# LANL-Bioinformatics/KWAGE

Hardware: AMD Instinct MI355X
Metric: G k-mer·sample bit-tests/sec (+ achieved HBM GB/s of the gather kernel in `roofline`) (higher is better)
Workload: dtype u32

## Files before the change

kwage_amd/csrc/engine.hip:

```cpp
#include <hip/hip_runtime.h>
#include <hip/hip_ext.h>

#include <algorithm>
#include <chrono>
#include <cmath>
#include <cstdio>
#include <cctype>
#include <cstring>
#include <new>
#include <string>
#include <thread>
#include <vector>

#include <unistd.h>

#include "host.hpp"
#include "engine_state.hpp"
#include "kernels.hpp"
#include "search_plan.hpp"

using namespace kwage;


struct TuningName { const char *name; int64_t Tuning::*field; };
static const TuningName TUNING_NAMES[] = {
	{"walk", &Tuning::walk}, {"walk_min_rows", &Tuning::walk_min_rows}, {"walk_max_kib", &Tuning::walk_max_kib}, {"walk_min_kib", &Tuning::walk_min_kib}, {"walk_tile_kib", &Tuning::walk_tile_kib},
	 {"walk_waves", &Tuning::walk_waves}, {"walk_one_wg_per_cu", &Tuning::walk_one_wg_per_cu},
	{"walk_bands", &Tuning::walk_bands}, {"walk_bands_min_gib", &Tuning::walk_bands_min_gib},
	{"and_vec", &Tuning::and_vec}, {"and_wide", &Tuning::and_wide}, {"and_wide_min_kib", &Tuning::and_wide_min_kib}, {"narrow", &Tuning::narrow}, {"force_segs", &Tuning::force_segs}, {"scores_form", &Tuning::scores_form},
	{"ee_refine", &Tuning::ee_refine}, {"refine_seg_rows", &Tuning::refine_seg_rows}, {"refine_min_rows", &Tuning::refine_min_rows}, {"refine_max_groups", &Tuning::refine_max_groups}, {"refine_unroll", &Tuning::refine_unroll}, {"refine_list_cap", &Tuning::refine_list_cap}, {"refine_static", &Tuning::refine_static}, {"screen_wpc", &Tuning::screen_wpc}, {"count_screen_wpc", &Tuning::count_screen_wpc}, {"count_screen_min_tiles", &Tuning::count_screen_min_tiles}, {"count_screen_check", &Tuning::count_screen_check}, {"count_trunc", &Tuning::count_trunc},
	{"count_walk", &Tuning::count_walk}, {"count_walk_wpc", &Tuning::count_walk_wpc}, {"count_walk_waves", &Tuning::count_walk_waves},
	{"count_walk_min_rows", &Tuning::count_walk_min_rows},
	{"hit_sort_host", &Tuning::hit_sort_host}, {"hit_copy_piece_kb", &Tuning::hit_copy_piece_kb}, {"shared_table_log2", &Tuning::shared_table_log2},
	{"ext_launch_events", &Tuning::ext_launch_events}, {"group_contiguous", &Tuning::group_contiguous}, {"group_placement_probe", &Tuning::group_placement_probe},
};

namespace kwage {

__global__ __launch_bounds__(KM_THREADS) void kmer_kernel(KmerArgs a)
{
	extern __shared__ __attribute__((aligned(16))) unsigned long long lds_tab[];
	__shared__ uint8_t codes[KM_THREADS + KWAGE_MAX_WORD_LEN];
	__shared__ uint32_t count, tile_base;

	const uint32_t q = a.chunk_q ? a.chunk_q[blockIdx.x] : blockIdx.x;
	const uint64_t t_begin = a.chunk_q ? a.chunk_t0[blockIdx.x] : 0;
	const uint64_t s0 = a.seq_off[q];
	const uint64_t len = a.seq_off[q + 1] - s0;
	const uint64_t npos = (len >= a.k) ? (len - a.k + 1) : 0;

	if(npos == 0){
		if(threadIdx.x == 0){ a.nkmer[q] = 0; a.qthr[q] = 0; }
		return;
// ... 26 lines not shown
{
	const uint32_t q = blockIdx.x / wgs_per_query, part = blockIdx.x % wgs_per_query;
	uint32_t *rq = rows + pos_off[q]*num_hash;
	const uint64_t n = (uint64_t)nkmer[q]*num_hash;
	for(uint64_t e = (uint64_t)part*blockDim.x + threadIdx.x; e < n; e += (uint64_t)wgs_per_query*blockDim.x){
		const uint32_t r = rq[e];
		uint32_t lo = 0, hi = map_len;
		while(lo < hi){
			const uint32_t mid = lo + (hi - lo)/2;
			if(map[mid] < r){ lo = mid + 1; } else { hi = mid; }
		}
		if(lo < map_len && map[lo] == r){ rq[e] = lo; }
		else{ rq[e] = 0; atomicAdd(missing, 1ull); }
	}
}

__global__ __launch_bounds__(SEARCH_THREADS) void and_refine_emit_kernel(SearchArgs a, RefineArgs ra)
{
	constexpr int B = 4;
	__shared__ WaveHitBuf hit_bufs[SEARCH_THREADS/WAVE];
	WaveHitBuf *hbuf = &hit_bufs[threadIdx.x >> 6];
	WaveHitState hst;
	const uint32_t lane = threadIdx.x & (WAVE - 1), l = lane & 7u, g = lane >> 3;
	const uint32_t n_clusters = refine_list_end(ra, 0);
	const uint32_t gw = __builtin_amdgcn_readfirstlane(blockIdx.x*(blockDim.x/WAVE) + (threadIdx.x >> 6));
	const uint32_t nw = gridDim.x*(blockDim.x/WAVE);
	for(uint64_t c0 = gw; c0 < n_clusters; c0 += (uint64_t)B*nw){
		RefineCluster cl[B];
		u32x4 m[B];
#pragma unroll
		for(int k = 0; k < B; ++k){
			const uint64_t ci = c0 + (uint64_t)k*nw;
			cl[k].q = REFINE_NONE;
			if(ci < n_clusters){ cl[k] = ra.clusters[ci]; }
		}
#pragma unroll
		for(int k = 0; k < B; ++k){
			const uint32_t groups = cl[k].kstep_groups & 0xFFu;
			m[k] = (u32x4)(0u);
			if(cl[k].q != REFINE_NONE && ((groups >> g) & 1u)){
				const uint32_t it = cl[k].first_item + __popc(groups & ((1u << g) - 1u));
				m[k] = reinterpret_cast<const u32x4*>(ra.masks)[(uint64_t)it*8 + l];
			}
		}
#pragma unroll
		for(int k = 0; k < B; ++k){
			if(cl[k].q == REFINE_NONE){ continue; }
			const uint32_t kstep = cl[k].kstep_groups >> 8;
			emit_masked_hits_buffered(a, hbuf, hst, cl[k].q, kstep*WAVE + lane, m[k], cl[k].n, (uint64_t)cl[k].q*a.runs_per_query + kstep);
		}
	}
	wave_hits_flush(a, hbuf, hst);
}

__global__ __launch_bounds__(256) void band_bucket_kernel(const uint32_t *__restrict__ rows, const uint64_t *__restrict__ pos_off, const uint32_t *__restrict__ nkmer,
                                                         uint32_t num_hash, uint32_t bands, uint32_t rows_per_band, uint32_t *__restrict__ loc, uint32_t *__restrict__ rows2)
{
// ... 328 lines not shown
}

int launch_count_combine(const SearchPlan &p, const SearchArgs &a, hipStream_t s, const StageEvents &ge)
{
	return by_planes(p.planes, [&](auto P) -> int {
		constexpr int PLANES = decltype(P)::value;
		constexpr size_t lds = (size_t)(COMBINE_WAVES/2)*PLANES*WAVE*16;
		int rc;
		if((rc = allow_dynamic_lds(count_combine_kernel<PLANES>, lds))){ return rc; }
		KW_GATHER_LAUNCH(ge, false, true, (count_combine_kernel<PLANES>), dim3(p.combine_wgs, a.n_queries), dim3(COMBINE_WAVES*WAVE), lds, s, a, p.seg_planes);
		return KWAGE_OK;
	});
}

int reserve_zeroed(DevBuf &buf, uint64_t bytes, hipStream_t s)
{
	if(bytes <= buf.cap){ return KWAGE_OK; }
	int rc = buf.reserve(bytes);
	if(rc){ return rc; }
	HIP_TRY(hipMemsetAsync(buf.p, 0, buf.cap, s));
	return KWAGE_OK;
}

int refine_setup(Slot *sl, const RefinePlan &r, hipStream_t gs, RefineArgs *out)
{
	int rc;
	RefineArgs &ra = *out;
	auto list = [](const ListPlan &l) { return RefineList{l.cap, l.stat, l.base, l.chunk}; };
	ra.seg_rows = r.seg_rows;
	ra.min_rows = r.min_rows;
	ra.max_groups = r.max_groups;
	ra.lc = list(r.lc);
	ra.li = list(r.li);
	ra.lu = list(r.lu);
	if((rc = sl->ref_counters.reserve(8*sizeof(uint32_t)))){ return rc; }
	if((rc = sl->ref_clusters.reserve(r.clusters*sizeof(RefineCluster)))){ return rc; }
	if((rc = sl->ref_masks.reserve(r.items*r.item_bytes))){ return rc; }
	if((rc = sl->ref_units.reserve(r.units*sizeof(RefineUnit)))){ return rc; }
	if(r.unit_bytes && (rc = sl->ref_slab.reserve(r.units*r.unit_bytes))){ return rc; }
	ra.counters = (uint32_t*)sl->ref_counters.p;
	ra.clusters = (RefineCluster*)sl->ref_clusters.p;
	ra.masks = (uint32_t*)sl->ref_masks.p;
	ra.units = (RefineUnit*)sl->ref_units.p;
	ra.slab = (uint32_t*)sl->ref_slab.p;
	HIP_TRY(hipMemsetAsync(ra.counters, 0, 8*sizeof(uint32_t), gs));
	sl->ref_base[0] = ra.lc.base; sl->ref_base[1] = ra.li.base; sl->ref_base[2] = ra.lu.base;
	sl->ref_cap[0] = ra.lc.cap; sl->ref_cap[1] = ra.li.cap; sl->ref_cap[2] = ra.lu.cap;
	ra.queue_batch = r.queue_batch;
	ra.check_every = r.check_every;
	return KWAGE_OK;
}

int count_walk_setup(Slot *sl, const SearchPlan &p, hipStream_t gs, CountWalkArgs *wa)
{
	int rc;
	wa->total_slots = p.total_slots;
	wa->per_wave = p.per_wave;
	wa->coltiles = p.chunks;
	if((rc = sl->cwalk_slab.reserve(p.exchange_bytes))){ return rc; }
	if((rc = reserve_zeroed(sl->cwalk_arrived, p.flags_bytes, gs))){ return rc; }
	wa->slab = (uint32_t*)sl->cwalk_slab.p;
	wa->arrived = (uint32_t*)sl->cwalk_arrived.p;
	wa->slot_off = nullptr; wa->kcut = nullptr;
	return KWAGE_OK;
}

uint32_t count_screen_blocks_per_cu(uint32_t planes, uint32_t nh)
{
	static int cache[3][5] = {};
	const int pi = (planes <= 7) ? 0 : (planes <= 10) ? 1 : 2, ni = (int)std::min(std::max(nh, 1u), 5u) - 1;
// ... 198 lines not shown
static const uint64_t SORT_SCRATCH_KEEP = 1ull << 30;

struct SearchOutcome {
	uint64_t staged_hits = 0;
	uint64_t n_hits = 0;
	uint64_t total_kmers = 0;
	float kmer_ms = 0, search_ms = 0;
	uint32_t launches = 0;
	char kernel_name[64] = "";
};

int enqueue_search_and_copy(Slot *sl)
{
	int rc;
	kwage_group *g = sl->g;
	kwage_batch *b = sl->b;
	const bool timing = (sl->flags & KWAGE_SEARCH_TIMING) != 0;
	const bool own = (sl->ext_hits == nullptr && sl->ext_cap == 0);
	const uint64_t cap = own ? sl->hit_cap : sl->ext_cap;
	kwage_hit *d_hits = own ? sl->d_hits : sl->ext_hits;
	if(b->n && g->num_columns){
		hipStream_t gs = g->ctx->gather_stream;
		if(sl->n_runs){ HIP_TRY(hipMemsetAsync(sl->runs.p, 0, sl->n_runs*sizeof(unsigned long long), sl->stream)); }
		HIP_TRY(hipEventRecord(sl->kmer_done, sl->stream));
		HIP_TRY(hipStreamWaitEvent(gs, sl->kmer_done, 0));
		if(sl->append && sl->append_reset){ HIP_TRY(hipMemsetAsync(sl->ext_count, 0, sizeof(uint64_t), gs)); }
		const bool ride = g->ctx->tune.ext_launch_events != 0;
		StageEvents ge;
		if(ride){ ge.start = timing ? sl->ev[2] : nullptr; ge.stop = sl->gather_done; }
		else if(timing){ HIP_TRY(hipEventRecord(sl->ev[2], gs)); }
		unsigned long long *hit_count = sl->append ? (unsigned long long*)sl->ext_count : (unsigned long long*)sl->d_counters;
		if((rc = launch_search_stage(sl, g, b, sl->lay, sl->threshold, sl->flags, d_hits, cap, hit_count, gs, ge))){ return rc; }
		if(!ride){ HIP_TRY(hipEventRecord(sl->gather_done, gs)); }
		HIP_TRY(hipStreamWaitEvent(sl->stream, sl->gather_done, 0));
		++sl->launches;
	}
	else if(sl->append && sl->append_reset){
		hipStream_t gs = g->ctx->gather_stream;
		HIP_TRY(hipMemsetAsync(sl->ext_count, 0, sizeof(uint64_t), gs));
		HIP_TRY(hipEventRecord(sl->gather_done, gs));
		HIP_TRY(hipStreamWaitEvent(sl->stream, sl->gather_done, 0));
	}
	if(sl->append){
		HIP_TRY(hipMemcpyAsync(sl->d_counters, sl->ext_count, sizeof(uint64_t), hipMemcpyDeviceToDevice, sl->stream));
	}
	else if(sl->ext_count){
// ... 172 lines not shown
			hipLaunchKernelGGL(count_nonzero_kernel, dim3((uint32_t)std::min<uint64_t>(2048, (n + 255)/256)), dim3(256), 0, ctx->stream,
			                   (const uint32_t*)bufs[j]->p, n, d + j);
		}
		e = hipGetLastError();
	}
	unsigned long long h[5] = {0, 0, 0, 0, 0};
	if(e == hipSuccess){ e = hipMemcpyAsync(h, d, sizeof(h), hipMemcpyDeviceToHost, ctx->stream); }
	if(e == hipSuccess){ e = hipStreamSynchronize(ctx->stream); }
	(void)hipFree(d);
	if(e != hipSuccess){ return fail(KWAGE_ERR_DEVICE, "kwage_ctx_scratch_nonzero: %s", hipGetErrorString(e)); }
	for(int j = 0; j < 5; ++j){ out[j] = h[j]; }
	return KWAGE_OK;
}

extern "C" int kwage_ctx_refine_stats(kwage_ctx *ctx, uint64_t out[8])
{
	if(!ctx || !out){ return fail(KWAGE_ERR_ARG, "kwage_ctx_refine_stats: NULL argument"); }
	for(int i = 0; i < 2; ++i){ if(ctx->slot[i].busy){ return fail(KWAGE_ERR_STATE, "kwage_ctx_refine_stats: a search is pending on this context"); } }
	int rc = set_device(ctx);
	if(rc){ return rc; }
	HIP_TRY(hipStreamSynchronize(ctx->gather_stream));
	for(int k = 0; k < 2; ++k){
		Slot *sl = &ctx->slot[k];
		uint32_t h[4] = {0, 0, 0, 0};
		if(sl->ref_counters.p){ HIP_TRY(hipMemcpy(h, sl->ref_counters.p, sizeof(h), hipMemcpyDeviceToHost)); }
		for(int j = 0; j < 3; ++j){ out[4*k + j] = std::min<uint64_t>((uint64_t)sl->ref_base[j] + h[j], sl->ref_cap[j]); }
		out[4*k + 3] = sl->ref_cap[2];
	}
	return KWAGE_OK;
}

namespace kwage {
hipStream_t ctx_stream(kwage_ctx *ctx) { return ctx->stream; }
int ctx_device(kwage_ctx *ctx) { return ctx->device; }
}

extern "C" int kwage_device_count(void)
{
	int n = 0;
	if(hipGetDeviceCount(&n) != hipSuccess){ return 0; }
	return n;
}

extern "C" int kwage_init(int device, kwage_ctx **out)
{
	if(!out){ return fail(KWAGE_ERR_ARG, "kwage_init: out is NULL"); }
// ... 610 lines not shown
```

kwage_amd/csrc/engine_state.hpp:

```cpp
#ifndef KWAGE_AMD_ENGINE_STATE_HPP
#define KWAGE_AMD_ENGINE_STATE_HPP

#include <hip/hip_runtime.h>

#include <algorithm>
#include <deque>
#include <memory>
#include <mutex>
#include <type_traits>
#include <vector>

#include "internal.h"
#include "tuning.hpp"

#define HIP_TRY(expr)                                                                          \
	do {                                                                                       \
		hipError_t _e = (expr);                                                                \
		if(_e != hipSuccess){                                                                  \
			return fail(KWAGE_ERR_DEVICE, "%s failed: %s (%s:%d)", #expr, hipGetErrorString(_e), \
			            __FILE__, __LINE__);                                                   \
		}                                                                                      \
	} while(0)

struct kwage_group;
// ... 183 lines not shown
	uint32_t *d_nkmer = nullptr, *d_qthr = nullptr;
	kwage_hit *d_hits = nullptr;
	uint64_t hit_cap = 0, head_bytes = 0;
	PinBuf h_stage;
	DevBuf sort_scratch;
	DevBuf runs;
	uint64_t n_runs = 0;
	uint32_t runs_per_query = 0;
	bool busy = false;
	kwage_group *g = nullptr;
	kwage_batch *b = nullptr;
	const KmerLayout *lay = nullptr;
	float threshold = 1.0f;
	uint32_t flags = 0;
	uint32_t launches = 0;
	char kernel_name[64] = "";
	DevBuf walk_or, walk_done;
	DevBuf band_rows, band_loc, band_or, band_state;
	DevBuf cwalk_slab, cwalk_arrived;
	DevBuf ref_counters, ref_clusters, ref_masks, ref_units, ref_slab;
	DevBuf trunc_dev;
	PinBuf trunc_host;
	uint32_t ref_base[3] = {0, 0, 0}, ref_cap[3] = {0, 0, 0};
	uint64_t staged_hits = 0;
	kwage_hit *ext_hits = nullptr;
	uint64_t ext_cap = 0;
	uint64_t *ext_count = nullptr;
	bool append = false, append_reset = false;
	uint32_t col_base = 0;
};

}

struct kwage_ctx {
	int device = -1;
	int ncu = 0;
	kwage::Tuning tune;
	hipStream_t stream = nullptr;
	hipStream_t gather_stream = nullptr;
	hipStream_t upload_stream = nullptr;
	kwage::Slot slot[2];
	kwage::DevBuf kmers;
	kwage::DevPool batch_pool;
	kwage::PinBuf load_pin[2];
	kwage::DevBuf load_dev[3];
	hipEvent_t load_done[3] = {nullptr, nullptr, nullptr};
// ... 169 lines not shown
```

kwage_amd/csrc/kernels.hpp:

```cpp
#ifndef KWAGE_AMD_KERNELS_HPP
#define KWAGE_AMD_KERNELS_HPP

#include <hip/hip_runtime.h>
#include <stdint.h>

#include "kwage_amd.h"
#include "kmer_device.hpp"
#include "tuning.hpp"

namespace kwage {

static constexpr int KM_THREADS = 256;
static constexpr uint32_t KM_LDS_SLOTS = 4096;
static constexpr uint32_t KM_CHUNK = 1024;
static constexpr uint64_t KM_EMPTY = ~0ull;


__device__ __forceinline__ uint32_t table_log2(uint64_t npos)
{
	uint32_t lg = 6;
	while((1ull << lg) < 2*npos){ ++lg; }
	return lg;
}

template <typename PTR>
__device__ __forceinline__ bool set_insert(PTR tab, uint32_t lg, uint64_t w)
{
	const uint64_t mask = (1ull << lg) - 1ull;
	uint64_t s = ((w * 0x9E3779B97F4A7C15ull) >> (64 - lg)) & mask;
	while(true){
// ... 399 lines not shown
	}
}

struct RefineUnit { uint32_t item, r0, r1, unit0, rq_lo, rq_hi, q, pad; };
struct RefineCluster {
	uint32_t q, kstep_groups, first_item, n;
	uint32_t first_unit, nseg, pad0, pad1;
};
static constexpr uint32_t REFINE_NONE = 0xFFFFFFFFu;

struct RefineList { uint32_t cap, stat, base, chunk; };
struct RefineArgs {
	uint32_t *counters;
	RefineCluster *clusters;
	uint32_t *masks;
	RefineUnit *units;
	uint32_t *slab;
	RefineList lc, li, lu;
	uint32_t seg_rows;
	uint32_t min_rows;
	uint32_t max_groups;
	uint32_t queue_batch;
	uint32_t check_every;
};

__device__ __forceinline__ uint32_t group_bits(uint64_t lanes)
{
	uint32_t g = 0;
#pragma unroll
	for(int k = 0; k < 8; ++k){ g |= ((lanes >> (8*k)) & 0xFFull) ? (1u << k) : 0u; }
	return g;
}

__device__ __forceinline__ uint32_t nth_set_bit(uint32_t bits, uint32_t j)
{
	for(uint32_t k = 0; k < j; ++k){ bits &= bits - 1; }
	return __ffs(bits) - 1;
}

struct RefineChunk { uint32_t next = 0, end = 0; };

__device__ __forceinline__ void refine_none_clusters(const RefineArgs &ra, uint32_t from, uint32_t to)
{
	to = min(to, ra.lc.cap);
	for(uint32_t i = from + (threadIdx.x & (WAVE - 1)); i < to; i += WAVE){ ra.clusters[i].q = REFINE_NONE; }
}
// ... 14 lines not shown
		uint32_t r = 0;
		if((threadIdx.x & (WAVE - 1)) == 0){ r = atomicAdd(ra.counters + which, want); }
		const uint64_t at = (uint64_t)ls.base + __builtin_amdgcn_readfirstlane(r);
		if(at + want > ls.cap){
			if(at < ls.cap){
				if(which == 0){ refine_none_clusters(ra, (uint32_t)at, ls.cap); } else if(which == 2){ refine_none_units(ra, (uint32_t)at, ls.cap); }
			}
			return REFINE_NONE;
		}
		ch.next = (uint32_t)at;
		ch.end = (uint32_t)at + want;
	}
	const uint32_t at = ch.next;
	ch.next += need;
	return at;
}

__device__ __forceinline__ uint32_t refine_list_end(const RefineArgs &ra, int which)
{
	const RefineList &ls = (which == 0) ? ra.lc : (which == 1) ? ra.li : ra.lu;
	return (uint32_t)min((uint64_t)ls.base + ra.counters[which], (uint64_t)ls.cap);
}

template <int VEC, int UNROLL>
__global__ __launch_bounds__(SEARCH_THREADS) void and_screen_kernel(SearchArgs a, RefineArgs ra)
{
	const uint32_t lane = threadIdx.x & (WAVE - 1);
	const uint64_t n_tiles = (uint64_t)a.n_queries*a.chunks;
	const uint32_t n_waves = gridDim.x*(blockDim.x/WAVE);
	const uint32_t gw = __builtin_amdgcn_readfirstlane(blockIdx.x*(blockDim.x/WAVE) + (threadIdx.x >> 6));
	__shared__ WaveHitBuf hit_bufs[SEARCH_THREADS/WAVE];
	WaveHitBuf *hbuf = &hit_bufs[threadIdx.x >> 6];
	WaveHitState hst;
	RefineChunk cc, ci, cu;
	cc.next = gw*ra.lc.stat; cc.end = cc.next + ra.lc.stat;
	ci.next = gw*ra.li.stat; ci.end = ci.next + ra.li.stat;
	cu.next = gw*ra.lu.stat; cu.end = cu.next + ra.lu.stat;
	bool lists_full = false;
	for(uint64_t tile = gw; tile < n_tiles; tile += n_waves){
		const uint32_t q = __builtin_amdgcn_readfirstlane((uint32_t)(tile / a.chunks));
		const uint32_t c = __builtin_amdgcn_readfirstlane((uint32_t)(tile % a.chunks));
		const uint32_t n = a.nkmer[q];
		if(n == 0){ continue; }
		const uint32_t nrows = n*a.num_hash;
		const uint64_t rq_off = a.pos_off[q]*a.num_hash;
		const uint32_t *rq = a.rows + rq_off;

		uint32_t unit[VEC];
		u32x4 acc[VEC];
#pragma unroll
		for(int v = 0; v < VEC; ++v){
			const uint32_t u = c*(WAVE*VEC) + v*WAVE + lane;
			const bool live = (u < a.units_per_row);
			unit[v] = live ? u : (a.units_per_row - 1);
			acc[v] = live ? reinterpret_cast<const u32x4*>(a.valid)[u] : (u32x4)(0u);
		}

		bool may_hand_over = !lists_full, gone = false;
		uint32_t i = 0;
		for(; i + UNROLL <= nrows; i += UNROLL){
// ... 5 lines not shown
#pragma unroll
				for(int v = 0; v < VEC; ++v){ x[u][v] = load16<true>(p + unit[v]); }
			}
#pragma unroll
			for(int u = 0; u < UNROLL; ++u){
#pragma unroll
				for(int v = 0; v < VEC; ++v){ acc[v] &= x[u][v]; }
			}
			uint32_t gb[VEC], ngroups = 0;
#pragma unroll
			for(int v = 0; v < VEC; ++v){
				gb[v] = group_bits(__ballot((acc[v].x | acc[v].y | acc[v].z | acc[v].w) != 0));
				ngroups += __popc(gb[v]);
			}
			if(ngroups == 0){ gone = true; break; }
			const uint32_t done = i + UNROLL;
			if(may_hand_over && ngroups <= ra.max_groups && nrows - done >= ra.min_rows && (done >= 2*UNROLL || nrows < 4*ra.seg_rows)){
				may_hand_over = false;
				const uint32_t nseg = (nrows - done + ra.seg_rows - 1)/ra.seg_rows;
				uint32_t nc = 0;
#pragma unroll
				for(int v = 0; v < VEC; ++v){ nc += gb[v] ? 1u : 0u; }
				const uint32_t nu = ngroups*nseg;
				const uint32_t c0 = refine_take(ra, 0, cc, nc);
				const uint32_t i0 = (c0 != REFINE_NONE) ? refine_take(ra, 1, ci, ngroups) : REFINE_NONE;
				const uint32_t u0 = (i0 != REFINE_NONE) ? refine_take(ra, 2, cu, nu) : REFINE_NONE;
				if(u0 == REFINE_NONE){
					if(c0 != REFINE_NONE){ refine_none_clusters(ra, c0, c0 + nc); }
					lists_full = true;
					continue;
				}
				uint32_t cidx = c0, ii = i0, all_groups = 0;
#pragma unroll
				for(int v = 0; v < VEC; ++v){
					all_groups |= gb[v] << (8*v);
					if(!gb[v]){ continue; }
					if(lane == 0){
						RefineCluster cl; cl.q = q; cl.kstep_groups = ((c*VEC + v) << 8) | gb[v]; cl.first_item = ii; cl.n = n;
						cl.first_unit = 0; cl.nseg = 0; cl.pad0 = 0; cl.pad1 = 0;
						ra.clusters[cidx] = cl;
					}
					const uint32_t k = lane >> 3;
					if((gb[v] >> k) & 1u){
						const uint32_t it = ii + __popc(gb[v] & ((1u << k) - 1u));
						reinterpret_cast<u32x4*>(ra.masks)[(uint64_t)it*8 + (lane & 7u)] = acc[v];
					}
					++cidx;
					ii += __popc(gb[v]);
				}
				for(uint32_t e = lane; e < nu; e += WAVE){
					const uint32_t j = e / nseg, sg = e % nseg;
					const uint32_t gpos = nth_set_bit(all_groups, j);
					RefineUnit un;
					un.item = i0 + j;
					un.r0 = done + sg*ra.seg_rows;
					un.r1 = min(nrows, un.r0 + ra.seg_rows);
					un.unit0 = c*(WAVE*VEC) + gpos*8u;
					un.rq_lo = (uint32_t)rq_off; un.rq_hi = (uint32_t)(rq_off >> 32);
					un.q = q; un.pad = 0;
					ra.units[u0 + e] = un;
				}
				gone = true;
				break;
			}
		}
		if(gone){ continue; }
		for(; i < nrows; ++i){
			const uint32_t r = rq[i];
			const u32x4 *p = reinterpret_cast<const u32x4*>(a.db + (uint64_t)r*a.stride);
#pragma unroll
			for(int v = 0; v < VEC; ++v){ acc[v] &= load16<true>(p + unit[v]); }
		}
#pragma unroll
		for(int v = 0; v < VEC; ++v){
			emit_masked_hits_buffered(a, hbuf, hst, q, unit[v], acc[v], n, (uint64_t)q*a.runs_per_query + c*VEC + v);
		}
	}
	wave_hits_flush(a, hbuf, hst);
	refine_none_clusters(ra, cc.next, cc.end);
	refine_none_units(ra, cu.next, cu.end);
}

template <int UNROLL>
__global__ __launch_bounds__(SEARCH_THREADS) void and_refine_kernel(SearchArgs a, RefineArgs ra)
{
	static_assert(UNROLL == 8 || UNROLL == 16, "eight or sixteen rows in flight");
	const uint32_t lane = threadIdx.x & (WAVE - 1), l = lane & 7u, sh = lane & ~7u;
	const uint32_t n_units = refine_list_end(ra, 2);
	const uint64_t gw = (uint64_t)blockIdx.x*(blockDim.x/WAVE) + (threadIdx.x >> 6);
	const uint64_t step = (uint64_t)gridDim.x*(blockDim.x/WAVE)*8;
	for(uint64_t base = gw*8; base < n_units; base += step){
		const uint64_t u = base + (lane >> 3);
		RefineUnit un;
		un.item = REFINE_NONE;
		if(u < n_units){ un = ra.units[u]; }
		bool on = (un.item != REFINE_NONE);
		uint32_t *M = ra.masks;
		u32x4 m = (u32x4)(0u);
		if(on){
			M = ra.masks + ((uint64_t)un.item*8 + l)*4;
#pragma unroll
			for(int d = 0; d < 4; ++d){ m[d] = __hip_atomic_load(M + d, __ATOMIC_RELAXED, __HIP_MEMORY_SCOPE_AGENT); }
		}
		on = on && (((uint32_t)(__ballot((m.x | m.y | m.z | m.w) != 0) >> sh) & 0xFFu) != 0);
		if(on){
			const uint32_t *rq = a.rows + (((uint64_t)un.rq_hi << 32) | un.rq_lo);
			const u32x4 *col = reinterpret_cast<const u32x4*>(a.db) + (un.unit0 + l);
			u32x4 acc = ~(u32x4)(0u);
			bool alive = true;
			for(uint32_t b = un.r0; alive && b < un.r1; b += 64){
				uint32_t idx[8];
#pragma unroll
				for(int k = 0; k < 8; ++k){ idx[k] = rq[min(b + 8u*k + l, un.r1 - 1)]; }
#pragma unroll
				for(int k = 0; k < 8; k += UNROLL/8){
					if(b + 8u*k >= un.r1){ break; }
					u32x4 x[UNROLL];
#pragma unroll
// ... 1081 lines not shown
```

kwage_amd/csrc/search_plan.hpp:

```cpp
#ifndef KWAGE_AMD_SEARCH_PLAN_HPP
#define KWAGE_AMD_SEARCH_PLAN_HPP

#include <algorithm>
#include <cmath>
#include <cstdint>
#include <cstdio>

#include "internal.h"
#include "tuning.hpp"

namespace kwage {

inline uint32_t planes_for(uint64_t max_count)
{
	uint32_t bits = 1;
	while(bits < 32 && (max_count >> bits) != 0){ ++bits; }
	return (bits <= 7) ? 7 : (bits <= 10) ? 10 : (bits <= 14) ? 14 : (bits <= 20) ? 20 : 32;
}

struct Segments { uint32_t segs, seg_kmers; };
inline Segments choose_segments(uint64_t n_queries, uint32_t chunks, uint64_t max_kmers, uint64_t max_segs, int64_t force_segs)
{
	static const uint64_t TARGET_TILES = 2048, MIN_SEG_KMERS = 64;
	Segments s = {1, (uint32_t)std::max<uint64_t>(max_kmers, 1)};
	uint64_t want = 1;
	if(force_segs > 0){ want = (uint64_t)force_segs; }
	else{
		const uint64_t tiles = n_queries*chunks;
		if(tiles >= TARGET_TILES || max_kmers < 2*MIN_SEG_KMERS){ return s; }
		want = std::min<uint64_t>((TARGET_TILES + tiles - 1)/tiles, max_kmers/MIN_SEG_KMERS);
	}
// ... 18 lines not shown
};

struct SearchInputs {
	uint64_t ncu = 1;
	uint64_t stride = 0, nrows = 0;
	uint32_t num_hash = 1;
	uint64_t alloc_bytes = 0;
	bool mixes_regions = false;
	double density_max = 1.0;
	uint32_t n_queries = 0;
	uint64_t total_pos = 0, max_pos = 0;
	const uint64_t *h_pos_off = nullptr;
	float threshold = 1.0f;
	uint32_t flags = 0;
	uint32_t (*count_screen_blocks_per_cu)(uint32_t planes, uint32_t nh) = nullptr;
};

struct ListPlan { uint32_t cap, stat, base, chunk; };
struct RefinePlan {
	uint32_t seg_rows = 0, min_rows = 0, max_groups = 0, queue_batch = 0, check_every = 0;
	ListPlan lc = {}, li = {}, lu = {};
	uint64_t clusters = 0, items = 0, units = 0, item_bytes = 0, unit_bytes = 0;
	uint32_t refine_wgs = 0, emit_wgs = 0;
};

struct SearchPlan {
	SearchForm form = SearchForm::AND_TILED;
	int vec = 0, unroll = 0, up = 0;
	uint32_t ch = 0, G = 0, planes = 0, seg_planes = 0, tplanes = 0;
	uint32_t nh = 0, num_hash = 0;
	uint32_t segs = 1, seg_kmers = 0, chunks = 0;
	uint32_t wgs = 0, wg_waves = 0;
	size_t lds = 0;
	uint32_t combine_wgs = 0;
	uint32_t finish_wgs = 0;
	uint32_t bands = 0, rows_per_band = 0;
	uint64_t total_slots = 0, per_wave = 0;
	RefinePlan refine;
	uint64_t partial_bytes = 0;
	uint64_t exchange_bytes = 0;
	uint64_t flags_bytes = 0;
	uint64_t band_rows_bytes = 0, band_loc_bytes = 0;
	uint64_t trunc_bytes = 0;
	double trunc_pm = 0;
	uint64_t seg = 0;
};
// ... 35 lines not shown

inline AndCfg and_config(const Tuning &t, uint32_t units_per_row, bool wide = false)
{
	AndCfg c;
	if(wide && t.and_vec == 0){ c.vec = 4; c.lds_bytes = 80*1024; return c; }
	c.vec = (t.and_vec == 1 || t.and_vec == 2 || t.and_vec == 4) ? (int)t.and_vec : ((units_per_row >= 4*WAVE) ? 2 : 1);
	c.lds_bytes = 0;
	return c;
}

inline int check_refine_units(uint32_t planes, int up)
{
	if(up == 14 && planes < 14){ return fail(KWAGE_ERR_STATE, "count refine: 14-plane units with %u counter planes", planes); }
	return KWAGE_OK;
}

inline uint32_t refine_unit_len(const Tuning &tn)
{
	return (uint32_t)std::min<int64_t>(std::max<int64_t>(tn.refine_seg_rows, 8), 120)/8*8;
}

inline void refine_plan(const Tuning &tn, uint32_t n_queries, uint64_t total_rows, uint64_t max_rows, uint32_t max_seg, uint64_t item_bytes, uint64_t unit_bytes,
                        uint64_t tiles, uint64_t screen_waves, uint64_t ncu, RefinePlan &r,
                        uint64_t exact_clusters = 0, uint64_t exact_items = 0, uint64_t exact_units = 0)
{
	r.seg_rows = (uint32_t)std::min<int64_t>(std::max<int64_t>(tn.refine_seg_rows, 8), max_seg);
	r.seg_rows = (uint32_t)std::max<uint64_t>(r.seg_rows, (max_rows + 65535)/65536);
	r.min_rows = (uint32_t)std::max<int64_t>(tn.refine_min_rows, 1);
	r.max_groups = (uint32_t)std::min<int64_t>(std::max<int64_t>(tn.refine_max_groups, 0), 16);
	uint64_t items = std::min<uint64_t>(std::max<uint64_t>(8ull*n_queries, 1u << 16), 1u << 20);
	items = std::max<uint64_t>(std::min<uint64_t>(items, (256ull << 20)/item_bytes), 1024);
	uint64_t units = std::min<uint64_t>(std::max<uint64_t>(32*total_rows/r.seg_rows, 1u << 18), 1u << 25);
	if(unit_bytes){ units = std::max<uint64_t>(std::min<uint64_t>(units, (512ull << 20)/unit_bytes), 4096); }
	if(tn.refine_list_cap > 0){ items = units = (uint64_t)std::min<int64_t>(tn.refine_list_cap, 1 << 20); }
	uint64_t clusters = items;
	if(exact_units){ clusters = exact_clusters; items = exact_items; units = exact_units; }
	if(exact_units && tn.refine_list_cap > 0){ clusters = items = units = (uint64_t)std::min<int64_t>(tn.refine_list_cap, 1 << 20); }
	const uint64_t tiles_per_wave = (tiles + screen_waves - 1)/std::max<uint64_t>(screen_waves, 1);
	auto list = [&](uint64_t cap, uint64_t stat_max, uint64_t chunk_max) {
		ListPlan ls;
		ls.cap = (uint32_t)cap;
		ls.stat = (tn.refine_static && !exact_units) ? (uint32_t)std::min<uint64_t>(stat_max, cap/2/std::max<uint64_t>(screen_waves, 1)) : 0u;
		ls.base = (uint32_t)(ls.stat*screen_waves);
		ls.chunk = exact_units ? 1u : (uint32_t)std::max<uint64_t>(1, std::min<uint64_t>(chunk_max, tiles_per_wave/4));
		return ls;
	};
	r.lc = list(clusters, 32, 32);
	r.li = list(items, 64, 64);
	r.lu = list(units, 256, 256);
	r.clusters = clusters; r.items = items; r.units = units;
	r.item_bytes = item_bytes; r.unit_bytes = unit_bytes;
	r.queue_batch = (uint32_t)std::max<uint64_t>(1, std::min<uint64_t>(16, tiles/(8*std::max<uint64_t>(screen_waves, 1))));
	r.check_every = (tn.count_screen_check == 16 || tn.count_screen_check == 32 || tn.count_screen_check == 64) ? (uint32_t)tn.count_screen_check : 8u;
	r.refine_wgs = (uint32_t)(ncu*8);
	r.emit_wgs = (uint32_t)(ncu*4);
}

inline int plan_and(const Tuning &tn, const SearchInputs &in, SearchPlan &p)
{
	const uint64_t ncu = std::max<uint64_t>(in.ncu, 1), n = in.n_queries;
	const uint32_t units_per_row = (uint32_t)(in.stride/16);
	const bool early_exit = (in.flags & KWAGE_SEARCH_EARLY_EXIT) != 0;
	const uint32_t whole_list = (uint32_t)std::max<uint64_t>(in.max_pos, 1);
	int rc;
	const uint64_t wide_tiles = n*((units_per_row + 4*WAVE - 1)/(4*WAVE));
	const bool wide_ok = tn.and_wide && !early_exit && wide_tiles >= 8*ncu;
	const bool wide_rows = wide_ok && units_per_row > (uint32_t)std::max<int64_t>(tn.and_wide_min_kib, 1)*WAVE;
	const AndCfg cfg = and_config(tn, units_per_row, wide_rows);
	p.chunks = (units_per_row + WAVE*cfg.vec - 1)/(WAVE*cfg.vec);
	const Segments sg = choose_segments(n, p.chunks, in.max_pos, max_segments(n, 4096), tn.force_segs);
	p.segs = sg.segs; p.seg_kmers = sg.seg_kmers;
	if((rc = check_launch_size(n, p.segs, p.chunks))){ return rc; }
	if(tn.narrow && p.segs == 1 && units_per_row <= 32 && n >= 64){
		p.form = SearchForm::AND_NARROW;
		p.G = (units_per_row <= 4) ? 16 : (units_per_row <= 8) ? 8 : (units_per_row <= 16) ? 4 : 2;
		const uint64_t waves = (n + p.G - 1)/p.G;
		p.wgs = (uint32_t)((waves + 3)/4); p.wg_waves = SEARCH_THREADS/WAVE;
		p.unroll = (waves < ncu*16) ? 16 : 8;
		return KWAGE_OK;
	}
	if(early_exit && tn.ee_refine && units_per_row >= WAVE && tn.force_segs <= 0){
		p.form = SearchForm::AND_SCREEN;
		p.vec = (units_per_row >= 4*WAVE) ? 2 : 1;
		p.segs = 1; p.seg_kmers = whole_list;
		p.chunks = (units_per_row + WAVE*p.vec - 1)/(WAVE*p.vec);
		const uint64_t tiles = n*p.chunks;
		const uint64_t screen_waves = (std::min<uint64_t>(tiles, ncu*(uint64_t)std::max<int64_t>(tn.screen_wpc, 1)) + 3)/4*4;
		refine_plan(tn, in.n_queries, in.total_pos*in.num_hash, in.max_pos*in.num_hash, 1u << 20, 128, 0, tiles, screen_waves, ncu, p.refine);
		p.unroll = (tn.refine_unroll == 16) ? 16 : 8;
		p.wgs = (uint32_t)(screen_waves/4); p.wg_waves = SEARCH_THREADS/WAVE;
		return KWAGE_OK;
	}
	const uint64_t walk_min_rows = (tn.walk_min_rows >= 0) ? (uint64_t)tn.walk_min_rows : (uint64_t)WALK_MIN_ROWS_PER_WAVE*256*WALK_WAVES_PER_CU;
	const uint32_t kib = (units_per_row + WAVE - 1)/WAVE;
	const uint32_t walk_max_kib = (uint32_t)std::max<int64_t>(tn.walk_max_kib, 0);
	const uint32_t walk_tile = (uint32_t)std::min<int64_t>(std::max<int64_t>(tn.walk_tile_kib, 1), 16);
	const uint32_t coltiles = (kib + walk_tile - 1)/walk_tile, walk_ch = (kib + coltiles - 1)/coltiles;
	const bool walk_ee_ok = !early_exit;
	const uint64_t walk_slots = (uint64_t)coltiles*in.total_pos;
	const uint32_t walk_min_kib = (uint32_t)std::max<int64_t>(tn.walk_min_kib, 1);
	if(tn.walk && walk_ee_ok && kib >= walk_min_kib && kib <= walk_max_kib && walk_slots*in.num_hash >= walk_min_rows && walk_slots > 0){
		const uint64_t waves = set_persistent(p, tn, persistent_waves(tn.walk_waves, ncu*WALK_WAVES_PER_CU, walk_slots, in.num_hash), ncu, walk_slots);
		p.ch = walk_ch;
		p.segs = 1; p.seg_kmers = whole_list;
		p.chunks = coltiles;
		const uint64_t band_items = in.total_pos*in.num_hash;
		const bool big_enough = in.alloc_bytes >= ((uint64_t)std::max<int64_t>(tn.walk_bands_min_gib, 0) << 30);
		const uint32_t bands = !big_enough ? 0u : (tn.walk_bands < 0) ? (in.mixes_regions ? 3u : 0u) : (uint32_t)std::min<int64_t>(tn.walk_bands, BAND_MAX);
		if(bands >= 2 && coltiles == 1 && walk_ch >= 3 && n*16*1024 <= (256ull << 20) && band_items < 0x7FFFFFFFull){
			p.form = SearchForm::AND_BAND_WALK;
			p.unroll = 4;
// ... 197 lines not shown
```

kwage_amd/csrc/tuning.hpp:

```cpp
#ifndef KWAGE_AMD_TUNING_HPP
#define KWAGE_AMD_TUNING_HPP

#include <cstdint>

namespace kwage {

static constexpr int WAVE = 64;
static constexpr int SEARCH_THREADS = 256;
static constexpr int WALK_WG_WAVES = 8;
static constexpr uint32_t BAND_MAX = 64;
static constexpr uint32_t CWALK_LEVELS = 32;
static constexpr uint32_t REFINE_UNIT_BYTES = 32;

struct Tuning {
	int64_t walk = 4;
	int64_t walk_min_rows = -1;
	int64_t walk_max_kib = 16;
	int64_t walk_tile_kib = 16;
	int64_t walk_min_kib = 2;
	int64_t walk_waves = 0;
	int64_t walk_one_wg_per_cu = 1;
	int64_t walk_bands = -1;
	int64_t walk_bands_min_gib = 48;
	int64_t and_vec = 0;
	int64_t and_wide_min_kib = 16;
	int64_t and_wide = 1;
	int64_t narrow = 1;
	int64_t force_segs = 0;
	int64_t scores_form = 0;
	int64_t ee_refine = 1;
	int64_t refine_seg_rows = 32;
	int64_t refine_min_rows = 32;
	int64_t refine_max_groups = 4;
	int64_t refine_unroll = 8;
	int64_t screen_wpc = 20;
	int64_t count_screen_wpc = 32;
	int64_t count_screen_min_tiles = 8192;
	int64_t count_trunc = 1;
	int64_t count_screen_check = 8;
	int64_t refine_static = 1;
	int64_t refine_list_cap = 0;
	int64_t count_walk = 1;
	int64_t count_walk_wpc = 8;
	int64_t count_walk_waves = 0;
	int64_t count_walk_min_rows = -1;
	int64_t hit_sort_host = 0;
	int64_t hit_copy_piece_kb = 0;
	int64_t ext_launch_events = 1;
	int64_t shared_table_log2 = 0;
	int64_t group_contiguous = 1;
	int64_t group_placement_probe = 1;
};

}

#endif
```

Measured before the change: 52260.

## Shard early-exit refine lists into per-segment counters with packed atomic reservation

Replaces the single global refine-list counters (chunked takes per wave) with up to 256 sharded segments, each with its own cache-line counter. Screen waves reserve cluster, item and unit slots in their own segment with one packed 64-bit atomic where the counts fit. The refine and emit kernels build a per-block prefix table over segment fill levels and map task indices to segments by binary search. The aim is to cut contention on the global atomics, at the cost of an extra memset, an LDS scan per block, and possible per-shard overflow when the load is uneven.

```diff
diff --git a/kwage_amd/csrc/engine.hip b/kwage_amd/csrc/engine.hip
--- a/kwage_amd/csrc/engine.hip
+++ b/kwage_amd/csrc/engine.hip
@@ -28,7 +28,7 @@
 	 {"walk_waves", &Tuning::walk_waves}, {"walk_one_wg_per_cu", &Tuning::walk_one_wg_per_cu},
 	{"walk_bands", &Tuning::walk_bands}, {"walk_bands_min_gib", &Tuning::walk_bands_min_gib},
 	{"and_vec", &Tuning::and_vec}, {"and_wide", &Tuning::and_wide}, {"and_wide_min_kib", &Tuning::and_wide_min_kib}, {"narrow", &Tuning::narrow}, {"force_segs", &Tuning::force_segs}, {"scores_form", &Tuning::scores_form},
-	{"ee_refine", &Tuning::ee_refine}, {"refine_seg_rows", &Tuning::refine_seg_rows}, {"refine_min_rows", &Tuning::refine_min_rows}, {"refine_max_groups", &Tuning::refine_max_groups}, {"refine_unroll", &Tuning::refine_unroll}, {"refine_list_cap", &Tuning::refine_list_cap}, {"refine_static", &Tuning::refine_static}, {"screen_wpc", &Tuning::screen_wpc}, {"count_screen_wpc", &Tuning::count_screen_wpc}, {"count_screen_min_tiles", &Tuning::count_screen_min_tiles}, {"count_screen_check", &Tuning::count_screen_check}, {"count_trunc", &Tuning::count_trunc},
+	{"ee_refine", &Tuning::ee_refine}, {"refine_seg_rows", &Tuning::refine_seg_rows}, {"refine_min_rows", &Tuning::refine_min_rows}, {"refine_max_groups", &Tuning::refine_max_groups}, {"refine_unroll", &Tuning::refine_unroll}, {"refine_list_cap", &Tuning::refine_list_cap}, {"refine_static", &Tuning::refine_static}, {"refine_shards", &Tuning::refine_shards}, {"screen_wpc", &Tuning::screen_wpc}, {"count_screen_wpc", &Tuning::count_screen_wpc}, {"count_screen_min_tiles", &Tuning::count_screen_min_tiles}, {"count_screen_check", &Tuning::count_screen_check}, {"count_trunc", &Tuning::count_trunc},
 	{"count_walk", &Tuning::count_walk}, {"count_walk_wpc", &Tuning::count_walk_wpc}, {"count_walk_waves", &Tuning::count_walk_waves},
 	{"count_walk_min_rows", &Tuning::count_walk_min_rows},
 	{"hit_sort_host", &Tuning::hit_sort_host}, {"hit_copy_piece_kb", &Tuning::hit_copy_piece_kb}, {"shared_table_log2", &Tuning::shared_table_log2},
@@ -101,7 +101,9 @@
 	WaveHitBuf *hbuf = &hit_bufs[threadIdx.x >> 6];
 	WaveHitState hst;
 	const uint32_t lane = threadIdx.x & (WAVE - 1), l = lane & 7u, g = lane >> 3;
-	const uint32_t n_clusters = refine_list_end(ra, 0);
+	__shared__ uint32_t pre[REFINE_MAX_SHARDS + 1], filled[REFINE_MAX_SHARDS], wave_sums[SEARCH_THREADS/WAVE];
+	refine_task_table(ra, 0, 1, pre, filled, wave_sums);
+	const uint32_t n_clusters = pre[ra.shards];
 	const uint32_t gw = __builtin_amdgcn_readfirstlane(blockIdx.x*(blockDim.x/WAVE) + (threadIdx.x >> 6));
 	const uint32_t nw = gridDim.x*(blockDim.x/WAVE);
 	for(uint64_t c0 = gw; c0 < n_clusters; c0 += (uint64_t)B*nw){
@@ -111,7 +113,10 @@
 		for(int k = 0; k < B; ++k){
 			const uint64_t ci = c0 + (uint64_t)k*nw;
 			cl[k].q = REFINE_NONE;
-			if(ci < n_clusters){ cl[k] = ra.clusters[ci]; }
+			if(ci < n_clusters){
+				const ShardTask tk = shard_task(pre, ra.shards, (uint32_t)ci);
+				cl[k] = ra.clusters[(uint64_t)tk.seg*ra.lc.chunk + tk.off];
+			}
 		}
 #pragma unroll
 		for(int k = 0; k < B; ++k){
@@ -486,6 +491,13 @@
 	return KWAGE_OK;
 }
 
+static const uint64_t REF_COUNTER_BYTES = (uint64_t)REFINE_MAX_SHARDS*REFINE_LINE_WORDS*sizeof(uint32_t);
+
+bool may_screen_and(const Tuning &tn, float threshold, uint32_t flags)
+{
+	return threshold == 1.0f && (flags & KWAGE_SEARCH_EARLY_EXIT) != 0 && tn.ee_refine && tn.force_segs <= 0;
+}
+
 int refine_setup(Slot *sl, const RefinePlan &r, hipStream_t gs, RefineArgs *out)
 {
 	int rc;
@@ -497,7 +509,13 @@
 	ra.lc = list(r.lc);
 	ra.li = list(r.li);
 	ra.lu = list(r.lu);
-	if((rc = sl->ref_counters.reserve(8*sizeof(uint32_t)))){ return rc; }
+	ra.shards = r.shards;
+	ra.packed = r.packed ? 1u : 0u;
+	if(r.shards){
+		if(!sl->ref_zeroed || sl->ref_counters.cap < REF_COUNTER_BYTES || r.shards > REFINE_MAX_SHARDS){ return fail(KWAGE_ERR_STATE, "early-exit search: the lists' counters were not zeroed before the stage"); }
+		sl->ref_zeroed = false;
+	}
+	else if((rc = sl->ref_counters.reserve(8*sizeof(uint32_t)))){ return rc; }
 	if((rc = sl->ref_clusters.reserve(r.clusters*sizeof(RefineCluster)))){ return rc; }
 	if((rc = sl->ref_masks.reserve(r.items*r.item_bytes))){ return rc; }
 	if((rc = sl->ref_units.reserve(r.units*sizeof(RefineUnit)))){ return rc; }
@@ -507,9 +525,11 @@
 	ra.masks = (uint32_t*)sl->ref_masks.p;
 	ra.units = (RefineUnit*)sl->ref_units.p;
 	ra.slab = (uint32_t*)sl->ref_slab.p;
-	HIP_TRY(hipMemsetAsync(ra.counters, 0, 8*sizeof(uint32_t), gs));
+	if(!r.shards){ HIP_TRY(hipMemsetAsync(ra.counters, 0, 8*sizeof(uint32_t), gs)); }
 	sl->ref_base[0] = ra.lc.base; sl->ref_base[1] = ra.li.base; sl->ref_base[2] = ra.lu.base;
 	sl->ref_cap[0] = ra.lc.cap; sl->ref_cap[1] = ra.li.cap; sl->ref_cap[2] = ra.lu.cap;
+	sl->ref_shards = r.shards; sl->ref_packed = r.packed;
+	sl->ref_seg_cap[0] = ra.lc.chunk; sl->ref_seg_cap[1] = ra.li.chunk; sl->ref_seg_cap[2] = ra.lu.chunk;
 	ra.queue_batch = r.queue_batch;
 	ra.check_every = r.check_every;
 	return KWAGE_OK;
@@ -754,6 +774,12 @@
 	if(b->n && g->num_columns){
 		hipStream_t gs = g->ctx->gather_stream;
 		if(sl->n_runs){ HIP_TRY(hipMemsetAsync(sl->runs.p, 0, sl->n_runs*sizeof(unsigned long long), sl->stream)); }
+		sl->ref_zeroed = false;
+		if(may_screen_and(g->ctx->tune, sl->threshold, sl->flags)){
+			if((rc = sl->ref_counters.reserve(REF_COUNTER_BYTES))){ return rc; }
+			HIP_TRY(hipMemsetAsync(sl->ref_counters.p, 0, REF_COUNTER_BYTES, sl->stream));
+			sl->ref_zeroed = true;
+		}
 		HIP_TRY(hipEventRecord(sl->kmer_done, sl->stream));
 		HIP_TRY(hipStreamWaitEvent(gs, sl->kmer_done, 0));
 		if(sl->append && sl->append_reset){ HIP_TRY(hipMemsetAsync(sl->ext_count, 0, sizeof(uint64_t), gs)); }
@@ -972,6 +998,18 @@
 	HIP_TRY(hipStreamSynchronize(ctx->gather_stream));
 	for(int k = 0; k < 2; ++k){
 		Slot *sl = &ctx->slot[k];
+		if(sl->ref_shards){
+			std::vector<uint32_t> lines((size_t)sl->ref_shards*REFINE_LINE_WORDS, 0u);
+			if(sl->ref_counters.p){ HIP_TRY(hipMemcpy(lines.data(), sl->ref_counters.p, lines.size()*sizeof(uint32_t), hipMemcpyDeviceToHost)); }
+			for(int j = 0; j < 3; ++j){ out[4*k + j] = 0; }
+			for(uint32_t s = 0; s < sl->ref_shards; ++s){
+				const uint32_t *w = &lines[(size_t)s*REFINE_LINE_WORDS];
+				const uint32_t n[3] = {sl->ref_packed ? (w[0] & 0xFFFFu) : w[0], sl->ref_packed ? (w[0] >> REFINE_PACK_ITEM_SHIFT) : w[1], sl->ref_packed ? w[1] : w[2]};
+				for(int j = 0; j < 3; ++j){ out[4*k + j] += shard_filled(n[j], sl->ref_seg_cap[j]); }
+			}
+			out[4*k + 3] = sl->ref_cap[2];
+			continue;
+		}
 		uint32_t h[4] = {0, 0, 0, 0};
 		if(sl->ref_counters.p){ HIP_TRY(hipMemcpy(h, sl->ref_counters.p, sizeof(h), hipMemcpyDeviceToHost)); }
 		for(int j = 0; j < 3; ++j){ out[4*k + j] = std::min<uint64_t>((uint64_t)sl->ref_base[j] + h[j], sl->ref_cap[j]); }
diff --git a/kwage_amd/csrc/engine_state.hpp b/kwage_amd/csrc/engine_state.hpp
--- a/kwage_amd/csrc/engine_state.hpp
+++ b/kwage_amd/csrc/engine_state.hpp
@@ -229,6 +229,9 @@
 	DevBuf trunc_dev;
 	PinBuf trunc_host;
 	uint32_t ref_base[3] = {0, 0, 0}, ref_cap[3] = {0, 0, 0};
+	uint32_t ref_shards = 0, ref_seg_cap[3] = {0, 0, 0};
+	bool ref_packed = false;
+	bool ref_zeroed = false;
 	uint64_t staged_hits = 0;
 	kwage_hit *ext_hits = nullptr;
 	uint64_t ext_cap = 0;
diff --git a/kwage_amd/csrc/kernels.hpp b/kwage_amd/csrc/kernels.hpp
--- a/kwage_amd/csrc/kernels.hpp
+++ b/kwage_amd/csrc/kernels.hpp
@@ -6,6 +6,7 @@
 
 #include "kwage_amd.h"
 #include "kmer_device.hpp"
+#include "refine_shards.hpp"
 #include "tuning.hpp"
 
 namespace kwage {
@@ -451,6 +452,7 @@
 	uint32_t max_groups;
 	uint32_t queue_batch;
 	uint32_t check_every;
+	uint32_t shards, packed;
 };
 
 __device__ __forceinline__ uint32_t group_bits(uint64_t lanes)
@@ -511,6 +513,78 @@
 	return (uint32_t)min((uint64_t)ls.base + ra.counters[which], (uint64_t)ls.cap);
 }
 
+struct RefineCounts { uint32_t c, i, u; };
+__device__ __forceinline__ RefineCounts refine_unpack(uint64_t w)
+{
+	RefineCounts n;
+	n.c = (uint32_t)w & 0xFFFFu; n.i = ((uint32_t)w >> REFINE_PACK_ITEM_SHIFT) & 0xFFFFu; n.u = (uint32_t)(w >> REFINE_PACK_UNIT_SHIFT);
+	return n;
+}
+__device__ __forceinline__ uint32_t refine_seg_filled(const RefineArgs &ra, uint32_t seg, int which)
+{
+	const uint32_t *line = ra.counters + (uint64_t)seg*REFINE_LINE_WORDS;
+	uint32_t n;
+	if(ra.packed){
+		const RefineCounts k = refine_unpack(*reinterpret_cast<const uint64_t*>(line));
+		n = (which == 0) ? k.c : k.u;
+	}
+	else{ n = line[which]; }
+	return shard_filled(n, (which == 0) ? ra.lc.chunk : ra.lu.chunk);
+}
+
+struct RefinePlaces { uint32_t c0, i0, u0; };
+__device__ __forceinline__ bool refine_reserve(const RefineArgs &ra, uint32_t seg, uint32_t nc, uint32_t ni, uint32_t nu, RefinePlaces &at)
+{
+	const uint32_t lane = threadIdx.x & (WAVE - 1);
+	uint32_t *line = ra.counters + (uint64_t)seg*REFINE_LINE_WORDS;
+	const uint32_t cap_c = ra.lc.chunk, cap_i = ra.li.chunk, cap_u = ra.lu.chunk;
+	RefineCounts r;
+	if(ra.packed){
+		const RefineCounts seen = refine_unpack(__hip_atomic_load(reinterpret_cast<uint64_t*>(line), __ATOMIC_RELAXED, __HIP_MEMORY_SCOPE_AGENT));
+		if((uint64_t)seen.c + nc > cap_c || (uint64_t)seen.i + ni > cap_i || (uint64_t)seen.u + nu > cap_u){ return false; }
+		unsigned long long w = 0;
+		if(lane == 0){
+			w = atomicAdd(reinterpret_cast<unsigned long long*>(line), (unsigned long long)nc | ((unsigned long long)ni << REFINE_PACK_ITEM_SHIFT) | ((unsigned long long)nu << REFINE_PACK_UNIT_SHIFT));
+		}
+		const uint32_t lo = __builtin_amdgcn_readfirstlane((uint32_t)w), hi = __builtin_amdgcn_readfirstlane((uint32_t)(w >> 32));
+		r = refine_unpack(((uint64_t)hi << 32) | lo);
+	}
+	else{
+		const uint32_t sc = __hip_atomic_load(line, __ATOMIC_RELAXED, __HIP_MEMORY_SCOPE_AGENT), si = __hip_atomic_load(line + 1, __ATOMIC_RELAXED, __HIP_MEMORY_SCOPE_AGENT),
+			su = __hip_atomic_load(line + 2, __ATOMIC_RELAXED, __HIP_MEMORY_SCOPE_AGENT);
+		if((uint64_t)sc + nc > cap_c || (uint64_t)si + ni > cap_i || (uint64_t)su + nu > cap_u){ return false; }
+		uint32_t v0 = 0, v1 = 0, v2 = 0;
+		if(lane == 0){ v0 = atomicAdd(line, nc); v1 = atomicAdd(line + 1, ni); v2 = atomicAdd(line + 2, nu); }
+		r.c = __builtin_amdgcn_readfirstlane(v0); r.i = __builtin_amdgcn_readfirstlane(v1); r.u = __builtin_amdgcn_readfirstlane(v2);
+	}
+	at.c0 = seg*cap_c + r.c; at.i0 = seg*cap_i + r.i; at.u0 = seg*cap_u + r.u;
+	if((uint64_t)r.c + nc <= cap_c && (uint64_t)r.i + ni <= cap_i && (uint64_t)r.u + nu <= cap_u){ return true; }
+	for(uint64_t e = (uint64_t)r.c + lane; e < min((uint64_t)r.c + nc, (uint64_t)cap_c); e += WAVE){ ra.clusters[(uint64_t)seg*cap_c + e].q = REFINE_NONE; }
+	for(uint64_t e = (uint64_t)r.u + lane; e < min((uint64_t)r.u + nu, (uint64_t)cap_u); e += WAVE){ ra.units[(uint64_t)seg*cap_u + e].item = REFINE_NONE; }
+	return false;
+}
+
+__device__ __forceinline__ void refine_task_table(const RefineArgs &ra, int which, uint32_t per, uint32_t *pre, uint32_t *filled, uint32_t *wave_sums)
+{
+	static_assert(SEARCH_THREADS >= (int)REFINE_MAX_SHARDS, "a thread per segment");
+	const uint32_t t = threadIdx.x, lane = t & (WAVE - 1);
+	const uint32_t f = (t < ra.shards) ? refine_seg_filled(ra, t, which) : 0u;
+	uint32_t incl = shard_tasks(f, per);
+#pragma unroll
+	for(int d = 1; d < WAVE; d *= 2){
+		const uint32_t o = __shfl_up(incl, d);
+		if(lane >= (uint32_t)d){ incl += o; }
+	}
+	if(lane == WAVE - 1){ wave_sums[t >> 6] = incl; }
+	if(t < REFINE_MAX_SHARDS){ filled[t] = f; }
+	__syncthreads();
+	uint32_t before = 0;
+	for(uint32_t w = 0; w < (t >> 6); ++w){ before += wave_sums[w]; }
+	if(t < REFINE_MAX_SHARDS){ pre[t + 1] = before + incl; }
+	if(t == 0){ pre[0] = 0; }
+	__syncthreads();
+}
+
 template <int VEC, int UNROLL>
 __global__ __launch_bounds__(SEARCH_THREADS) void and_screen_kernel(SearchArgs a, RefineArgs ra)
 {
@@ -521,10 +595,7 @@
 	__shared__ WaveHitBuf hit_bufs[SEARCH_THREADS/WAVE];
 	WaveHitBuf *hbuf = &hit_bufs[threadIdx.x >> 6];
 	WaveHitState hst;
-	RefineChunk cc, ci, cu;
-	cc.next = gw*ra.lc.stat; cc.end = cc.next + ra.lc.stat;
-	ci.next = gw*ra.li.stat; ci.end = ci.next + ra.li.stat;
-	cu.next = gw*ra.lu.stat; cu.end = cu.next + ra.lu.stat;
+	const uint32_t seg = gw & (ra.shards - 1);
 	bool lists_full = false;
 	for(uint64_t tile = gw; tile < n_tiles; tile += n_waves){
 		const uint32_t q = __builtin_amdgcn_readfirstlane((uint32_t)(tile / a.chunks));
@@ -576,15 +647,13 @@
 #pragma unroll
 				for(int v = 0; v < VEC; ++v){ nc += gb[v] ? 1u : 0u; }
 				const uint32_t nu = ngroups*nseg;
-				const uint32_t c0 = refine_take(ra, 0, cc, nc);
-				const uint32_t i0 = (c0 != REFINE_NONE) ? refine_take(ra, 1, ci, ngroups) : REFINE_NONE;
-				const uint32_t u0 = (i0 != REFINE_NONE) ? refine_take(ra, 2, cu, nu) : REFINE_NONE;
-				if(u0 == REFINE_NONE){
-					if(c0 != REFINE_NONE){ refine_none_clusters(ra, c0, c0 + nc); }
+				RefinePlaces at;
+				if(!refine_reserve(ra, seg, nc, ngroups, nu, at)){
 					lists_full = true;
 					continue;
 				}
-				uint32_t cidx = c0, ii = i0, all_groups = 0;
+				const uint32_t i0 = at.i0, u0 = at.u0;
+				uint32_t cidx = at.c0, ii = i0, all_groups = 0;
 #pragma unroll
 				for(int v = 0; v < VEC; ++v){
 					all_groups |= gb[v] << (8*v);
@@ -631,8 +700,6 @@
 		}
 	}
 	wave_hits_flush(a, hbuf, hst);
-	refine_none_clusters(ra, cc.next, cc.end);
-	refine_none_units(ra, cu.next, cu.end);
 }
 
 template <int UNROLL>
@@ -640,14 +707,17 @@
 {
 	static_assert(UNROLL == 8 || UNROLL == 16, "eight or sixteen rows in flight");
 	const uint32_t lane = threadIdx.x & (WAVE - 1), l = lane & 7u, sh = lane & ~7u;
-	const uint32_t n_units = refine_list_end(ra, 2);
-	const uint64_t gw = (uint64_t)blockIdx.x*(blockDim.x/WAVE) + (threadIdx.x >> 6);
-	const uint64_t step = (uint64_t)gridDim.x*(blockDim.x/WAVE)*8;
-	for(uint64_t base = gw*8; base < n_units; base += step){
-		const uint64_t u = base + (lane >> 3);
+	__shared__ uint32_t pre[REFINE_MAX_SHARDS + 1], filled[REFINE_MAX_SHARDS], wave_sums[SEARCH_THREADS/WAVE];
+	refine_task_table(ra, 2, REFINE_UNITS_PER_TASK, pre, filled, wave_sums);
+	const uint32_t n_tasks = pre[ra.shards];
+	const uint32_t gw = __builtin_amdgcn_readfirstlane(blockIdx.x*(blockDim.x/WAVE) + (threadIdx.x >> 6));
+	const uint32_t nw = gridDim.x*(blockDim.x/WAVE);
+	for(uint64_t task = gw; task < n_tasks; task += nw){
+		const ShardTask tk = shard_task(pre, ra.shards, (uint32_t)task);
+		const uint32_t place = tk.off*REFINE_UNITS_PER_TASK + (lane >> 3);
 		RefineUnit un;
 		un.item = REFINE_NONE;
-		if(u < n_units){ un = ra.units[u]; }
+		if(place < filled[tk.seg]){ un = ra.units[(uint64_t)tk.seg*ra.lu.chunk + place]; }
 		bool on = (un.item != REFINE_NONE);
 		uint32_t *M = ra.masks;
 		u32x4 m = (u32x4)(0u);
diff --git a/kwage_amd/csrc/refine_shards.hpp b/kwage_amd/csrc/refine_shards.hpp
--- /dev/null
+++ b/kwage_amd/csrc/refine_shards.hpp
@@ -0,0 +1,53 @@
+#ifndef KWAGE_AMD_REFINE_SHARDS_HPP
+#define KWAGE_AMD_REFINE_SHARDS_HPP
+
+#include <cstdint>
+
+#if defined(__HIPCC__)
+#define KWAGE_HD __host__ __device__
+#else
+#define KWAGE_HD
+#endif
+
+namespace kwage {
+
+static constexpr uint32_t REFINE_MAX_SHARDS = 256;
+static constexpr uint32_t REFINE_LINE_WORDS = 32;
+static constexpr uint32_t REFINE_UNITS_PER_TASK = 8;
+
+KWAGE_HD inline uint32_t shard_filled(uint32_t count, uint32_t cap) { return count < cap ? count : cap; }
+
+KWAGE_HD inline uint32_t shard_tasks(uint32_t filled, uint32_t per) { return (filled + per - 1)/per; }
+
+KWAGE_HD inline uint32_t pow2_floor(uint32_t v)
+{
+	uint32_t p = 1;
+	while(p <= v/2){ p *= 2; }
+	return p;
+}
+
+struct ShardTask { uint32_t seg, off; };
+KWAGE_HD inline ShardTask shard_task(const uint32_t *prefix, uint32_t S, uint32_t task)
+{
+	uint32_t lo = 0, hi = S;
+	while(hi - lo > 1){
+		const uint32_t mid = (lo + hi)/2;
+		if(prefix[mid] <= task){ lo = mid; } else { hi = mid; }
+	}
+	ShardTask t;
+	t.seg = lo;
+	t.off = task - prefix[lo];
+	return t;
+}
+
+static constexpr uint32_t REFINE_PACK_ITEM_SHIFT = 16, REFINE_PACK_UNIT_SHIFT = 32;
+KWAGE_HD inline bool shard_counts_pack(uint64_t cap_clusters, uint64_t cap_items, uint64_t cap_units, uint64_t waves_per_seg,
+                                       uint64_t need_clusters, uint64_t need_items, uint64_t need_units)
+{
+	return cap_clusters + waves_per_seg*need_clusters < (1ull << 16) && cap_items + waves_per_seg*need_items < (1ull << 16)
+		&& cap_units + waves_per_seg*need_units < (1ull << 32);
+}
+
+}
+
+#endif
diff --git a/kwage_amd/csrc/search_plan.hpp b/kwage_amd/csrc/search_plan.hpp
--- a/kwage_amd/csrc/search_plan.hpp
+++ b/kwage_amd/csrc/search_plan.hpp
@@ -7,6 +7,7 @@
 #include <cstdio>
 
 #include "internal.h"
+#include "refine_shards.hpp"
 #include "tuning.hpp"
 
 namespace kwage {
@@ -71,6 +72,8 @@
 	ListPlan lc = {}, li = {}, lu = {};
 	uint64_t clusters = 0, items = 0, units = 0, item_bytes = 0, unit_bytes = 0;
 	uint32_t refine_wgs = 0, emit_wgs = 0;
+	uint32_t shards = 0;
+	bool packed = false;
 };
 
 struct SearchPlan {
@@ -152,7 +155,7 @@
 
 inline void refine_plan(const Tuning &tn, uint32_t n_queries, uint64_t total_rows, uint64_t max_rows, uint32_t max_seg, uint64_t item_bytes, uint64_t unit_bytes,
                         uint64_t tiles, uint64_t screen_waves, uint64_t ncu, RefinePlan &r,
-                        uint64_t exact_clusters = 0, uint64_t exact_items = 0, uint64_t exact_units = 0)
+                        uint64_t exact_clusters = 0, uint64_t exact_items = 0, uint64_t exact_units = 0, bool dense = false)
 {
 	r.seg_rows = (uint32_t)std::min<int64_t>(std::max<int64_t>(tn.refine_seg_rows, 8), max_seg);
 	r.seg_rows = (uint32_t)std::max<uint64_t>(r.seg_rows, (max_rows + 65535)/65536);
@@ -178,6 +181,25 @@
 	r.lc = list(clusters, 32, 32);
 	r.li = list(items, 64, 64);
 	r.lu = list(units, 256, 256);
+	r.shards = 0; r.packed = false;
+	if(dense){
+		const uint64_t shortest = std::max<uint64_t>(1, std::min(clusters, std::min(items, units)));
+		const uint64_t groups = std::max<uint32_t>(r.max_groups, 1);
+		const uint64_t nseg_max = (max_rows + r.seg_rows - 1)/r.seg_rows + 1;
+		uint64_t S = 1;
+		if(tn.refine_shards > 0){ S = pow2_floor((uint32_t)std::min<uint64_t>(std::min<uint64_t>((uint64_t)tn.refine_shards, REFINE_MAX_SHARDS), shortest)); }
+		else if(tn.refine_static){
+			const uint64_t most = pow2_floor((uint32_t)std::min<uint64_t>(REFINE_MAX_SHARDS, std::max<uint64_t>(screen_waves, 1)));
+			while(S < most && clusters/(2*S) >= 16 && items/(2*S) >= 64 && units/(2*S) >= std::max<uint64_t>(256, 2*groups*nseg_max)){ S *= 2; }
+		}
+		auto segments = [&](uint64_t cap) { ListPlan ls; ls.cap = (uint32_t)cap; ls.stat = (uint32_t)S; ls.base = 0; ls.chunk = (uint32_t)(cap/S); return ls; };
+		r.lc = segments(clusters);
+		r.li = segments(items);
+		r.lu = segments(units);
+		r.shards = (uint32_t)S;
+		const uint64_t waves_per_seg = (std::max<uint64_t>(screen_waves, 1) + S - 1)/S;
+		r.packed = shard_counts_pack(r.lc.chunk, r.li.chunk, r.lu.chunk, waves_per_seg, 2, 16, 16*nseg_max);
+	}
 	r.clusters = clusters; r.items = items; r.units = units;
 	r.item_bytes = item_bytes; r.unit_bytes = unit_bytes;
 	r.queue_batch = (uint32_t)std::max<uint64_t>(1, std::min<uint64_t>(16, tiles/(8*std::max<uint64_t>(screen_waves, 1))));
@@ -216,7 +238,7 @@
 		p.chunks = (units_per_row + WAVE*p.vec - 1)/(WAVE*p.vec);
 		const uint64_t tiles = n*p.chunks;
 		const uint64_t screen_waves = (std::min<uint64_t>(tiles, ncu*(uint64_t)std::max<int64_t>(tn.screen_wpc, 1)) + 3)/4*4;
-		refine_plan(tn, in.n_queries, in.total_pos*in.num_hash, in.max_pos*in.num_hash, 1u << 20, 128, 0, tiles, screen_waves, ncu, p.refine);
+		refine_plan(tn, in.n_queries, in.total_pos*in.num_hash, in.max_pos*in.num_hash, 1u << 20, 128, 0, tiles, screen_waves, ncu, p.refine, 0, 0, 0, true);
 		p.unroll = (tn.refine_unroll == 16) ? 16 : 8;
 		p.wgs = (uint32_t)(screen_waves/4); p.wg_waves = SEARCH_THREADS/WAVE;
 		return KWAGE_OK;
diff --git a/kwage_amd/csrc/tuning.hpp b/kwage_amd/csrc/tuning.hpp
--- a/kwage_amd/csrc/tuning.hpp
+++ b/kwage_amd/csrc/tuning.hpp
@@ -39,6 +39,7 @@
 	int64_t count_trunc = 1;
 	int64_t count_screen_check = 8;
 	int64_t refine_static = 1;
+	int64_t refine_shards = 0;
 	int64_t refine_list_cap = 0;
 	int64_t count_walk = 1;
 	int64_t count_walk_wpc = 8;
```

Result: no change. 52220 (-0.1%).
